# rafayaamirgull/stereo_reconstruction_cv

Hardware: AMD Instinct MI355X
Metric: Mdisparities/s (higher is better)
Workload: dtype int16

## Files before the change

stereo_reconstruction_cv_amd/_lib.py:

```python
from __future__ import annotations

import ctypes as C
import os

_HERE = os.path.dirname(os.path.abspath(__file__))
LIB_PATH = os.environ.get("SGM_HIP_LIB") or os.path.join(_HERE, "csrc", "libsgm_hip.so")

SGM_OK = 0
SGM_TAP_COST, SGM_TAP_AGGR, SGM_TAP_DISP_RAW, SGM_TAP_DISP_MEDIAN = 0, 1, 2, 3
SGM_TAP_CONF_RAW, SGM_TAP_CONF = 4, 5
SGM_TAP_RIGHT_RAW, SGM_TAP_RIGHT = 6, 7
SGM_OPT_KEEP_AGGR, SGM_OPT_PROFILE, SGM_OPT_SCHEDULE, SGM_OPT_SWEEP_ROWS, SGM_OPT_PREPASS_ROWS, SGM_OPT_CHAIN_WGS, SGM_OPT_GROUP_MAX = 0, 1, 2, 3, 5, 6, 7
SGM_OPT_CHANNELS = 8
SGM_OPT_CONFIDENCE = 10
SGM_OPT_RIGHT_VIEW = 11
SGM_OPT_COST = 12
SGM_COST_BT, SGM_COST_CENSUS = 0, 1
SGM_OPT_DEBUG = 4
SGM_OPT_POISON = 9
SGM_DBG_VOXEL_TIGHT_TABLE, SGM_DBG_VOXEL_OTHER_REDUCTION = 1 << 22, 1 << 23
SGM_MAX_STAGES = 32

EXPORTS = (
    "sgm_abi_version", "sgm_device_count", "sgm_last_error", "sgm_create", "sgm_destroy",
    "sgm_set_option", "sgm_geometry", "sgm_compute", "sgm_compute_batch", "sgm_disp_to_float",
    "sgm_reproject", "sgm_valid_mask", "sgm_get_tap", "sgm_get_headroom", "sgm_median3x3", "sgm_filter_speckles", "sgm_compact_points",
    "sgm_compact_points_device", "sgm_compact_points_device_async", "sgm_compute_device", "sgm_check", "sgm_trim",
    "sgm_disp_to_float_device", "sgm_reproject_device", "sgm_valid_mask_device",
    "sgm_pipeline_device", "sgm_pipeline_batch_device", "sgm_synchronize", "sgm_get_stage_times", "sgm_algorithmic_bytes",
    "sgm_init_undistort_rectify_map", "sgm_init_undistort_rectify_map_device",
    "sgm_remap_linear_u8", "sgm_remap_linear_u8_device",
)
CONFIDENCE_EXPORTS = ("sgm_bind_confidence_device",)
RIGHT_EXPORTS = ("sgm_bind_right_device",)
WLS_EXPORTS = ("sgm_wls_weights", "sgm_wls_filter", "sgm_wls_filter_device")
WLS_BATCH_EXPORTS = ("sgm_wls_filter_batch", "sgm_wls_filter_batch_device")
LRC_EXPORTS = ("sgm_lrc_confidence", "sgm_lrc_confidence_device", "sgm_lrc_confidence_batch_device")
VOXEL_EXPORTS = ("sgm_voxel_downsample", "sgm_voxel_downsample_device")
MESH_EXPORTS = ("sgm_mesh_grid", "sgm_mesh_grid_device")


# ... 85 lines not shown
    L.sgm_mesh_grid_device.argtypes = [vp, vp, vp, vp, i32, i32, C.c_float, vp, vp, vp, vp, vp]
    L.sgm_synchronize.argtypes = [vp]
    L.sgm_get_stage_times.argtypes = [vp, C.POINTER(SgmStageTimes)]
    L.sgm_algorithmic_bytes.argtypes = [pp, i32, i32, i32]
    L.sgm_algorithmic_bytes.restype = i64
    L.sgm_init_undistort_rectify_map.argtypes = [vp, vp, vp, i32, vp, vp, i32, i32, i32, vp, vp]
    L.sgm_init_undistort_rectify_map_device.argtypes = [vp, vp, vp, i32, vp, vp, i32, i32, i32, vp, vp]
    L.sgm_remap_linear_u8.argtypes = [vp, vp, i32, i32, i64, i32, vp, vp, i32, i32, vp]
    L.sgm_remap_linear_u8_device.argtypes = [vp, vp, i32, i32, i64, i32, vp, vp, i32, i32, vp, i64]
    L.sgm_debug_plan.argtypes = [pp, i32, i32, i32, i32, i32, i32, i32, i32, C.POINTER(SgmDebugPlan)]
    L.sgm_debug_plan.restype = i32
    L.sgm_debug_plan_opts.argtypes = [pp, i32, i32, i32, i32, i32, i32, i32, i32, i32, i32, C.POINTER(SgmDebugPlan)]
    L.sgm_debug_plan_opts.restype = i32
    L.sgm_debug_plan_cost.argtypes = [pp, i32, i32, i32, i32, i32, i32, i32, i32, i32, i32, i32, C.POINTER(SgmDebugPlan)]
    L.sgm_debug_plan_cost.restype = i32
    L.sgm_debug_uniq_threshold.argtypes = [i32, i32]
    L.sgm_debug_uniq_threshold.restype = i32
    L.sgm_debug_wta_split.argtypes = [pp, i32, i32, i32, i32, i32, i32, i32, i32]
    L.sgm_debug_wta_split.restype = i32
    L.sgm_debug_wta_raw_bytes.argtypes = [vp]
    L.sgm_debug_wta_raw_bytes.restype = C.c_longlong
    L.sgm_debug_wta_select_n.argtypes = [i32, i32, vp, i32, vp]
    L.sgm_debug_wta_select_n.restype = i32
    for name in EXPORTS + CONFIDENCE_EXPORTS + RIGHT_EXPORTS + WLS_EXPORTS + WLS_BATCH_EXPORTS + LRC_EXPORTS + VOXEL_EXPORTS + MESH_EXPORTS:
        fn = getattr(L, name)
        if fn.restype is C.c_int and name not in ("sgm_abi_version", "sgm_device_count"):
            fn.restype = i32
    _lib = L
    return L


def last_error() -> str:
    return (load().sgm_last_error() or b"").decode("utf-8", "replace")


def debug_plan(params: dict, H: int, W: int, channels: int = 1, schedule: int = 1, sweep_rows: int = 0, prepass_rows: int = 0,
               debug: int = 0, frames: int = 1, confidence: int = 0, right_view: int = 0, cost: int = SGM_COST_BT) -> dict:
    out = SgmDebugPlan()
    if cost != SGM_COST_BT:
        rc = load().sgm_debug_plan_cost(C.byref(SgmParams(**params)), H, W, channels, schedule, sweep_rows, prepass_rows, debug,
                                        frames, confidence, right_view, cost, C.byref(out))
    elif confidence or right_view:
        rc = load().sgm_debug_plan_opts(C.byref(SgmParams(**params)), H, W, channels, schedule, sweep_rows, prepass_rows, debug,
                                        frames, confidence, right_view, C.byref(out))
    else:
        rc = load().sgm_debug_plan(C.byref(SgmParams(**params)), H, W, channels, schedule, sweep_rows, prepass_rows, debug, frames,
                                   C.byref(out))
    if rc != SGM_OK:
        raise ValueError(f"sgm_debug_plan failed ({rc}): {last_error()}")
    return {n: getattr(out, n) for n, _ in SgmDebugPlan._fields_}


def debug_wta_split(params: dict, H: int, W: int, schedule: int = 2, sweep_rows: int = 0, debug: int = 0, confidence: int = 0,
                    right_view: int = 0, keep_aggr: int = 0) -> bool:
    rc = load().sgm_debug_wta_split(C.byref(SgmParams(**params)), H, W, schedule, sweep_rows, debug, confidence, right_view, keep_aggr)
    if rc < 0:
        raise ValueError(f"sgm_debug_wta_split failed ({rc}): {last_error()}")
    return bool(rc)
```

stereo_reconstruction_cv_amd/csrc/kernels_sweep.h:

```cpp
#pragma once
#include "kernels_path.h"
#include <type_traits>

namespace sgm {

enum { SWEEP_FIRST = 0, SWEEP_ACCUM = 1, SWEEP_LAST = 2, SWEEP_REDUCE = 3 };

struct SweepArgs {
    int ydir, xdir;
    int R;
    const int16_t *C;
    int16_t *S;
    const int16_t *bndL;
    uint2 *wta;
    int keepS;
    int dbg;
    uint32_t *ctl;
    uint32_t *prog;
    uint32_t *err;
    int nbands;
};

constexpr int CHAIN_MAX_FRAMES = 64;
struct ChainFrames {
    int nf;
    const int16_t *C[CHAIN_MAX_FRAMES];
    int16_t *S[CHAIN_MAX_FRAMES];
    int16_t *bnd[CHAIN_MAX_FRAMES];
    uint32_t *hr[CHAIN_MAX_FRAMES];
    uint4 *raw[CHAIN_MAX_FRAMES];
};
static_assert(sizeof(Geom) + sizeof(SweepArgs) + sizeof(ChainFrames) + 64 <= 4096, "a kernel's arguments must stay within 4 KB");

constexpr int SWEEP_MAX_ROWS = 11;
__host__ __device__ constexpr int sweep_pps(int NP) { return NP == 4 ? 1 : (NP == 1 ? 4 : 2); }
__host__ __device__ constexpr int sweep_ring(int NP) { return 4 * sweep_pps(NP); }

__host__ __device__ constexpr int sweep_slot_dwords(int NP, int NR = 3) { return 64 * NR * NP; }
static inline size_t sweep_lds_bytes(int NP, int R, int NR = 3)
// ... 51 lines not shown
        until(need);
        pending = __hip_atomic_load(word, __ATOMIC_RELAXED, __HIP_MEMORY_SCOPE_AGENT);
    }
    __device__ __forceinline__ void until(uint32_t need)
    {
        if (seen >= need) return;
        uint32_t idle = 0, last = seen;
        for (;;) {
            seen = peek();
            if (seen >= need) break;
            __builtin_amdgcn_s_sleep(8);
            if (seen != last) {
                last = seen;
                idle = 0;
            } else if (++idle > CHAIN_GIVE_UP) {
                if (lane_id() == 0) atomicOr(err, 1u);
                seen = 0x7fffffffu;
                break;
            }
        }
    }
};

#ifndef SGM_CHAIN_HALF_BLOCKS
#define SGM_CHAIN_HALF_BLOCKS 0
#endif
template <int NP, bool PARTIAL, bool CHAIN, int NR = 3>
__device__ __forceinline__ void sweep_loader_wave(const Geom &g, const SweepArgs &a, int band, int lane, uint32_t *lds)
{
    constexpr int LDAUX = CHAIN ? 16 : (SGM_NT_SWEEP_LOADS ? 2 : 0);
    constexpr int PPS = sweep_pps(NP);
    constexpr int RING = sweep_ring(NP);
    constexpr int LB = (CHAIN && SGM_CHAIN_HALF_BLOCKS) ? RING / 2 : RING;
    constexpr int OFF_A = 0, OFF_B = LB % RING;
    static_assert(2 * PPS <= LB && LB % PPS == 0 && RING % LB == 0, "prologue writes 2 * PPS pixels of block 0");
    constexpr int SLOT = sweep_slot_dwords(NP, NR);
    constexpr int ROLE = 64 * NP;
    const int R = a.R;
    int W1 = g.W1;
    const int D = g.D;
    if (CHAIN) asm volatile("" : "+s"(W1));
    const int T = (W1 + PPS - 1) / PPS + 2 * (R - 1);
    const bool active = !PARTIAL || (2 * NP * lane < D);
    const int lane_off = active ? 2 * NP * lane : 0;
    const uint32_t init = active ? (CHAIN ? path_bias(g.P2) : 0u) : SGM_SENT;
    uint32_t *const ring0 = lds + lane * NP;

    const bool has_prev = band > 0 && !(a.dbg & 64);
    Pack<NP> bA[LB][NR], bB[LB][NR];
    const int row_bytes = W1 * NR * D * 2;
    const __amdgpu_buffer_rsrc_t rsrc = __builtin_amdgcn_make_buffer_rsrc(
        (void *)(a.bndL + (int64_t)band * W1 * NR * D), 0, row_bytes, 0x00020000);
    const int voff = lane_off * 2;
    const int px_bytes = NR * D * 2;
    const int pk = a.xdir > 0 ? px_bytes : -px_bytes;
    const int p0 = a.xdir > 0 ? 0 : (W1 - 1) * px_bytes;
    ChainWait cw;
    if (CHAIN && has_prev) {
        cw.word = a.prog + band - 1;
        cw.err = a.err;
    }
    auto lb_t = [&](auto full_c, Pack<NP>(*b)[NR], int k0) {
        constexpr bool FULL = decltype(full_c)::value;
        if (CHAIN) cw.step((uint32_t)min(k0 + LB, W1));
#pragma unroll
        for (int u = 0; u < LB; u++) {
            if (FULL || k0 + u < W1) {
                const int so = p0 + (k0 + u) * pk;
#pragma unroll
                for (int d = 0; d < NR; d++) buf_load<NP, LDAUX>(b[u][d], rsrc, voff, so + d * D * 2);
            }
        }
    };
    auto wb_t = [&](auto full_c, Pack<NP>(*b)[NR], int off, int u, int k) {
        constexpr bool FULL = decltype(full_c)::value;
// ... 363 lines not shown
            load_block_t(part, cB, sB, k0 + PB);
            compute_block_t(part, cA, sA, k0);
            load_block_t(part, cA, sA, k0 + 2 * PB);
            compute_block_t(part, cB, sB, k0 + PB);
        }
    }
    {
        const uint32_t hmax = wave_max_u32(hm) & 0xffffu;
        if (g.hr && lane == 0) headroom_raise(g.hr + 1, hmax);
    }
    if (wave < R - 1) {
        sweep_write_start_state<NP, NR>(mine, W1 % RING, init);
        for (int i = 0; i < 2 * (R - 1 - wave); i++) wg_barrier();
    }
}

template <int NP, bool PARTIAL, int MODE, bool POSW>
__global__ __launch_bounds__(SWEEP_MAX_ROWS * 64 + 64) void k_sweep(Geom g, SweepArgs a)
{
    extern __shared__ __attribute__((aligned(16))) uint32_t lds[];
    const int wave = __builtin_amdgcn_readfirstlane((int)(threadIdx.x >> 6));
    const int lane = threadIdx.x & 63;
    const int band = blockIdx.x;
    if (wave == a.R) sweep_loader_wave<NP, PARTIAL, false>(g, a, band, lane, lds);
    else sweep_compute_wave<NP, PARTIAL, MODE, POSW>(g, a, band, wave, lane, lds);
}

#ifndef SGM_CHAIN_KD
#define SGM_CHAIN_KD 3
#endif
constexpr int CHAIN_KD = SGM_CHAIN_KD;

template <int NP, bool PARTIAL, int NR = 3>
__device__ __forceinline__ void chain_publisher_wave(const Geom &g, const SweepArgs &a, int band, int lane, uint32_t *lds)
{
    constexpr int PPS = sweep_pps(NP);
    constexpr int RING = sweep_ring(NP);
    constexpr int SLOT = sweep_slot_dwords(NP, NR);
    constexpr int ROLE = 64 * NP;
    constexpr int STORES_PER_STEP = NR * PPS * (NP == 4 ? 2 : 1) + 1;
    static_assert(CHAIN_KD * STORES_PER_STEP <= 63, "vmcnt is a 6-bit counter");
    const int R = a.R;
    int W1 = g.W1;
    const int D = g.D;
    asm volatile("" : "+s"(W1));
    const int NS = (W1 + PPS - 1) / PPS;
    const int T = NS + 2 * (R - 1);
    const bool active = !PARTIAL || (2 * NP * lane < D);
    const int lane_off = active ? 2 * NP * lane : 0;
    const bool publishes = band + 1 < a.nbands;
    const uint32_t *const last = lds + lane * NP + R * RING * SLOT;
    const int row_bytes = W1 * NR * D * 2;
    const __amdgpu_buffer_rsrc_t rec = __builtin_amdgcn_make_buffer_rsrc(
        (void *)(a.bndL + (int64_t)(band + 1) * W1 * NR * D), 0, row_bytes, 0x00020000);
    const int voff = lane_off * 2;
    const int px_bytes = NR * D * 2;
    const int pk = a.xdir > 0 ? px_bytes : -px_bytes;
    const int p0 = a.xdir > 0 ? 0 : (W1 - 1) * px_bytes;
    uint32_t *const word = a.prog + band;
    if (!publishes) {
        for (int n = 0; n <= T; n++) wg_barrier();
        return;
    }
    for (int n = 0; n <= T + 1; n++) {
        const int i = n - 2 * (R - 1) - 2;
        if (i >= 0 && i < NS) {
#pragma unroll
            for (int p = 0; p < PPS; p++) {
                const int k = PPS * i + p;
                const uint32_t *s = last + (k % RING) * SLOT;
                Pack<NP> v[NR];
#pragma unroll
                for (int d = 0; d < NR; d++) lds_load<NP>(v[d], s + d * ROLE);
                const int so = k < W1 ? p0 + k * pk : row_bytes;
#pragma unroll
                for (int d = 0; d < NR; d++)
                    if (!PARTIAL || active) buf_store<NP, 16>(v[d], rec, voff, so + d * D * 2);
// ... 2 lines not shown
            Pack<NP> z;
            z.fill(0u);
#pragma unroll
            for (int p = 0; p < NR * PPS; p++)
                if (!PARTIAL || active) buf_store<NP, 16>(z, rec, voff, row_bytes);
        }
        __builtin_amdgcn_s_waitcnt(0x0f70 | ((CHAIN_KD * STORES_PER_STEP) & 15) | (((CHAIN_KD * STORES_PER_STEP) >> 4) << 14));
        const int done = min(max(PPS * (i - CHAIN_KD + 1), 0), W1);
        if (lane == 0) __hip_atomic_store(word, (uint32_t)done, __ATOMIC_RELAXED, __HIP_MEMORY_SCOPE_AGENT);
        if (n <= T) wg_barrier();
    }
    __builtin_amdgcn_s_waitcnt(0x0f70);
    if (lane == 0) __hip_atomic_store(word, (uint32_t)W1, __ATOMIC_RELAXED, __HIP_MEMORY_SCOPE_AGENT);
}

constexpr int CHAIN_MAX_ROWS = 12;
template <int NP, bool PARTIAL, int MODE>
__global__ __launch_bounds__(CHAIN_MAX_ROWS * 64 + 128) void k_sweep_chain(Geom g, SweepArgs a, ChainFrames fr)
{
    extern __shared__ __attribute__((aligned(16))) uint32_t lds[];
    const int wave = __builtin_amdgcn_readfirstlane((int)(threadIdx.x >> 6));
    const int lane = threadIdx.x & 63;
    uint32_t *const ticket = lds + (a.R + 1) * sweep_ring(NP) * sweep_slot_dwords(NP);
    for (;;) {
        if (threadIdx.x == 0) *ticket = atomicAdd(a.ctl, 1u);
        wg_barrier();
        const int tk = __builtin_amdgcn_readfirstlane((int)*ticket);
        if (tk >= a.nbands * fr.nf) break;
        const int f = tk % fr.nf, band = tk / fr.nf;
        a.C = fr.C[f];
        a.S = fr.S[f];
        a.bndL = fr.bnd[f];
        a.prog = a.ctl + 1 + f * a.nbands;
        g.hr = fr.hr[f];
        if constexpr (MODE == SWEEP_REDUCE) a.wta = reinterpret_cast<uint2 *>(fr.raw[f]);
        if (wave == a.R) sweep_loader_wave<NP, PARTIAL, true>(g, a, band, lane, lds);
        else if (wave == a.R + 1) chain_publisher_wave<NP, PARTIAL>(g, a, band, lane, lds);
        else sweep_compute_wave<NP, PARTIAL, MODE, true, 3, true>(g, a, band, wave, lane, lds);
    }
}

template <int NP, bool PARTIAL, int MODE>
__global__ __launch_bounds__(SWEEP_MAX_ROWS * 64 + 64) void k_axis_sweep(Geom g, SweepArgs a)
{
    static_assert(MODE == SWEEP_FIRST || MODE == SWEEP_ACCUM, "the axis-only sweeps have no fused winner-take-all");
    extern __shared__ __attribute__((aligned(16))) uint32_t lds[];
    const int wave = __builtin_amdgcn_readfirstlane((int)(threadIdx.x >> 6));
    const int lane = threadIdx.x & 63;
    const int band = blockIdx.x;
    if (wave == a.R) sweep_loader_wave<NP, PARTIAL, false, 1>(g, a, band, lane, lds);
    else sweep_compute_wave<NP, PARTIAL, MODE, true, 1>(g, a, band, wave, lane, lds);
}

template <int NP, bool PARTIAL, int MODE>
__global__ __launch_bounds__(CHAIN_MAX_ROWS * 64 + 128) void k_axis_chain(Geom g, SweepArgs a, ChainFrames fr)
{
    static_assert(MODE == SWEEP_FIRST || MODE == SWEEP_ACCUM, "the axis-only sweeps have no fused winner-take-all");
    extern __shared__ __attribute__((aligned(16))) uint32_t lds[];
    const int wave = __builtin_amdgcn_readfirstlane((int)(threadIdx.x >> 6));
    const int lane = threadIdx.x & 63;
    uint32_t *const ticket = lds + (a.R + 1) * sweep_ring(NP) * sweep_slot_dwords(NP, 1);
    for (;;) {
        if (threadIdx.x == 0) *ticket = atomicAdd(a.ctl, 1u);
        wg_barrier();
        const int tk = __builtin_amdgcn_readfirstlane((int)*ticket);
        if (tk >= a.nbands * fr.nf) break;
        const int f = tk % fr.nf, band = tk / fr.nf;
        a.C = fr.C[f];
        a.S = fr.S[f];
        a.bndL = fr.bnd[f];
        a.prog = a.ctl + 1 + f * a.nbands;
        g.hr = fr.hr[f];
        if (wave == a.R) sweep_loader_wave<NP, PARTIAL, true, 1>(g, a, band, lane, lds);
        else if (wave == a.R + 1) chain_publisher_wave<NP, PARTIAL, 1>(g, a, band, lane, lds);
        else sweep_compute_wave<NP, PARTIAL, MODE, true, 1, true>(g, a, band, wave, lane, lds);
    }
}

}
```

stereo_reconstruction_cv_amd/csrc/sgm_debug.h:

```cpp
#ifndef SGM_DEBUG_H
#define SGM_DEBUG_H

#define SGM_OPT_DEBUG 4

#define SGM_OPT_POISON 9

enum {
    SGM_DBG_WTA_IN_LAST_PATH = 2,
    SGM_DBG_NO_LANE_GROUPS = 4,
    SGM_DBG_NARROW_VSUM = 8,
    SGM_DBG_PREPASS_3_LAUNCHES = 16,
    SGM_DBG_NO_PREPASS_OVERLAP = 32,
    SGM_DBG_SKIP_BOUNDARY_LOADS = 64,
    SGM_DBG_FORK_PREPASS_EARLY = 128,
    SGM_DBG_INT16_COST = 256,
    SGM_DBG_PREPASS_ONE_CHUNK = 512,
    SGM_DBG_WTA_SEPARATE = 2048,
    SGM_DBG_SMALL_D_RECORD = 8192,
    SGM_DBG_IN_ROW_ON_MAIN_STREAM = 4096,
    SGM_DBG_FIFTH_PATH_AFTER_SWEEP = 65536,
    SGM_DBG_WLS_BATCH_ROWS_SHIFT = 17,
    SGM_DBG_WLS_BATCH_COLS_SHIFT = 20,
    SGM_DBG_VOXEL_TIGHT_TABLE = 1 << 22,
    SGM_DBG_VOXEL_OTHER_REDUCTION = 1 << 23
};

typedef struct {
    int W1, minX1, NP, partial;
    int byte_cost, pix_px, GWc, RBb, vsum_ring;
    int rows4, GWs, chain, R, nbands;
    int fused_prepass, prepass_g, pre_nch, pre_rows, overlap;
    int fused_wta, nvol, path_w_main, speckle;
    int chain_window;
} sgm_debug_plan_t;

#ifdef __cplusplus
extern "C"
#endif
int sgm_debug_plan(const sgm_params *p, int H, int W, int channels, int schedule, int sweep_rows, int prepass_rows,
                   int debug, int frames, sgm_debug_plan_t *out);
#ifdef __cplusplus
extern "C"
#endif
int sgm_debug_plan_opts(const sgm_params *p, int H, int W, int channels, int schedule, int sweep_rows, int prepass_rows,
                        int debug, int frames, int confidence, int right_view, sgm_debug_plan_t *out);
#ifdef __cplusplus
extern "C"
#endif
int sgm_debug_plan_cost(const sgm_params *p, int H, int W, int channels, int schedule, int sweep_rows, int prepass_rows,
                        int debug, int frames, int confidence, int right_view, int cost, sgm_debug_plan_t *out);

#ifdef __cplusplus
extern "C" {
#endif
int sgm_debug_uniq_threshold(int minS, int uniquenessRatio);
int sgm_debug_wta_split(const sgm_params *p, int H, int W, int schedule, int sweep_rows, int debug, int confidence, int right_view,
                        int keep_aggr);
long long sgm_debug_wta_raw_bytes(const sgm_engine *e);
int sgm_debug_wta_select_n(int D, int uniquenessRatio, const uint32_t *raw , int n, uint32_t *wta );
#ifdef __cplusplus
}
#endif

#endif
```

stereo_reconstruction_cv_amd/csrc/sgm_engine.hip:

```cpp
#include "../../include/sgm_hip.h"
#include "sgm_debug.h"

#include <hip/hip_runtime.h>

#include <dlfcn.h>

#include <algorithm>
#include <cmath>
#include <cstdarg>
#include <cstdio>
#include <cstdlib>
#include <cstring>
#include <string>
#include <thread>
#include <vector>

#include "kernels_cost.h"
#include "kernels_census.h"
#include "kernels_path.h"
#include "kernels_post.h"
#include "kernels_rectify.h"
#include "kernels_sweep.h"
#include "kernels_group.h"
#include "kernels_right.h"
// ... 145 lines not shown
        cap = bytes;
        return SGM_OK;
    }
    void release()
    {
        if (p) (void)hipHostFree(p);
        p = nullptr;
        cap = 0;
    }
};

struct Plan {
    bool byte_cost;
    bool pix_px;
    int GWc, RBb;
    bool vsum_ring, vsum_wide;
    int cn;
    bool census;
    bool v1;
    int GWs;
    bool rows4;
    bool chain;
    int npass, R, nbands;
    bool axis;
    int nroles;
    bool prepass_g;
    bool fused_prepass;
    bool pre_plain;
    int pre_nch, pre_rows;
    bool overlap, fork_early;
    bool fused_wta;
    bool wta_split;
    int nvol;
    bool path_w_main, path_w_lines;
    bool speckle;
};

#define SGM_ENGINE_DEVBUFS(BUF, ARR, MAP) \
    BUF(in_left) BUF(in_right)                    \
    BUF(lrec) BUF(rplanes)                        \
    BUF(hsum) BUF(cost) BUF(aggr)                 \
    BUF(aggr2) BUF(aggr3)                         \
    BUF(aggr4) BUF(aggr5)                         \
    BUF(wta)                                      \
    BUF(wta_raw)                                  \
    BUF(bndL) BUF(bndL2)                          \
// ... 349 lines not shown
    hipLaunchKernelGGL((k_sweep_chain<NP, PARTIAL, MODE>), dim3(wgs), dim3((a.R + 2) * 64), lds, st, g, a, fr);
    return SGM_OK;
}
template <int NP, bool PARTIAL>
static int launch_chain_np(const Geom &g, const SweepArgs &a, const ChainFrames &fr, int mode, int wgs, hipStream_t st)
{
    if (mode == SWEEP_FIRST) return launch_chain_one<NP, PARTIAL, SWEEP_FIRST>(g, a, fr, wgs, st);
    if constexpr (!PARTIAL && NP <= 2)
        if (mode == SWEEP_REDUCE) return launch_chain_one<NP, PARTIAL, SWEEP_REDUCE>(g, a, fr, wgs, st);
    if (mode == SWEEP_REDUCE) return set_err(SGM_ERR_INVALID_ARG, "internal: no SWEEP_REDUCE form of this chained sweep");
    return launch_chain_one<NP, PARTIAL, SWEEP_ACCUM>(g, a, fr, wgs, st);
}
static int launch_chain(const Geom &g, const SweepArgs &a, const ChainFrames &fr, int mode, int wgs, hipStream_t st, bool axis = false)
{
    if (int rc = check_sweep_direction(a, mode)) return rc;
    if (axis && mode == SWEEP_REDUCE) return set_err(SGM_ERR_INVALID_ARG, "internal: the axis-only sweeps have no SWEEP_REDUCE form");
    if (axis)
        return with_np(g, [&](auto np, auto part) {
            return mode == SWEEP_FIRST ? launch_axis_chain_one<np, part, SWEEP_FIRST>(g, a, fr, wgs, st)
                                       : launch_axis_chain_one<np, part, SWEEP_ACCUM>(g, a, fr, wgs, st);
        });
    return with_np(g, [&](auto np, auto part) { return launch_chain_np<np, part>(g, a, fr, mode, wgs, st); });
}
static int chain_window(const Geom &g, int R, int nbands, int nf, int override_wgs)
{
    const int pps = sweep_pps(g.NP);
    const int T = (g.W1 + pps - 1) / pps + 2 * (R - 1), lag = 2 * (R - 1) + 17;
    const int per_frame = override_wgs > 0 ? override_wgs : std::max(4, (T + lag - 1) / lag);
    return (int)std::min<int64_t>({(int64_t)per_frame * nf, (int64_t)nbands * nf, 256});
}

static int sweep_rows_for(const Geom &g, int override_rows, int npass, bool chained = false)
{
    int maxR = chained ? CHAIN_MAX_ROWS : SWEEP_MAX_ROWS;
    while (maxR > 1 && sweep_lds_bytes(g.NP, maxR) + 16 > 160 * 1024) maxR--;
    if (chained && override_rows <= 0) return std::max(1, std::min(maxR, g.H));
    const int bands = npass == 2 ? 200 : 240;
    int R = override_rows > 0 ? override_rows : (g.H + bands - 1) / bands;
    if (override_rows <= 0) R = std::max(R, 4);
    return std::max(1, std::min(R, maxR));
}

static int box_columns(int GW) { return 16 * (64 / GW); }

static Plan make_plan(const sgm_engine *e, const Geom &g, int H)
{
// ... 41 lines not shown
    p.wta_split = p.chain && g.mode == 1 && !p.axis && !p.fused_wta && !np_partial(g) && g.NP <= 2 && g.uniq < 100 &&
                  !e->keep_aggr && !e->no_wta_split && !conf && !(dbg & SGM_DBG_WTA_SEPARATE);
    const bool two_vol = g.mode == 0 && !p.fused_wta && !p.v1 && g.D <= 128 && !(dbg & SGM_DBG_NO_LANE_GROUPS) &&
                         !(dbg & SGM_DBG_FIFTH_PATH_AFTER_SWEEP);
    const bool three_vol = two_vol && p.rows4 && !(dbg & SGM_DBG_IN_ROW_ON_MAIN_STREAM);
    const bool five_vol = three_vol && !(dbg & SGM_DBG_SMALL_D_RECORD);
    p.nvol = five_vol ? 5 : three_vol ? 3 : two_vol ? 2 : 1;
    if (p.axis && p.rows4 && !p.v1) {
        p.nvol = 4;
        p.overlap = false;
    }
    p.path_w_main = !p.v1 && g.mode == 0 && p.nvol == 1;
    p.path_w_lines = (dbg & SGM_DBG_NO_LANE_GROUPS) != 0;
    p.speckle = e->params.speckleRange >= 0 && e->params.speckleWindowSize > 0;
    if (g.NP == 8) {
        p.v1 = true;
        p.byte_cost = p.pix_px = p.rows4 = p.chain = p.prepass_g = p.fused_prepass = false;
        p.overlap = p.fork_early = p.path_w_main = false;
        p.GWs = 64;
        p.fused_wta = !conf;
        p.wta_split = false;
        p.nvol = 1;
    }
    return p;
}

static int ensure_speckle_buffers(sgm_engine *e, size_t npx)
{
    int rc;
    if ((rc = e->label.ensure(npx * 4)) || (rc = e->csize.ensure(npx * 4))) return rc;
    return e->rlen.ensure(npx * 4);
}
static size_t chain_ctl_bytes(int nf, int nbands) { return ((size_t)(1 + (size_t)nf * nbands) * 4 + 15) & ~(size_t)15; }

static size_t plan_bytes_held(const sgm_engine *e)
{
    size_t n = 0;
    each_devbuf(e, [&](const DevBuf &b) { n += b.cap; });
    return n;
}
static int ensure_plan_buffers(sgm_engine *e, const Plan &p, int H, int W)
{
    Geom g;
    int rc = normalise(&e->params, H, W, &g);
    if (rc) return rc;
    e->g = g;
    e->H = H;
    e->W = W;
    const size_t npx = (size_t)H * W;
    const size_t vol = (size_t)std::max<int64_t>(g.rowsz, 0) * H * sizeof(int16_t);
    if ((rc = e->lrec.ensure(npx * 8 * p.cn + (debug_alloc_mode() ? 0 : 64)))) return rc;
    if ((rc = e->rplanes.ensure(p.census ? npx * 8 : npx * 6 * p.cn))) return rc;
    if (vol) {
        if (!p.byte_cost && (rc = e->hsum.ensure(vol))) return rc;
        if ((rc = e->cost.ensure(vol))) return rc;
        if ((rc = e->aggr.ensure(vol))) return rc;
        DevBuf *more[] = {&e->aggr2, &e->aggr3, &e->aggr4, &e->aggr5};
        for (int k = 1; k < p.nvol; k++)
            if ((rc = more[k - 1]->ensure(vol))) return rc;
    }
    if ((rc = e->wta.ensure(npx * 8))) return rc;
    if (p.wta_split && (rc = e->wta_raw.ensure(npx * 16))) return rc;
    if ((rc = e->disp_raw.ensure(npx * 2))) return rc;
    if ((rc = e->disp_med.ensure(npx * 2))) return rc;
    for (SideMap *m : {&e->conf, &e->right})
        if (m->on && ((rc = m->raw.ensure(npx * m->bpp)) || (rc = m->fin.ensure(npx * m->bpp)))) return rc;
    if (e->right.on && g.W1 > 0 && (rc = e->rrec.ensure((size_t)H * g.W1 * 8))) return rc;
    if ((rc = e->headroom.ensure(8))) return rc;
    e->g.hr = (uint32_t *)e->headroom.p;
    if (g.W1 > 0 && !p.v1 && p.nbands > 1 && p.nvol < 4) {
        const size_t bnd_bytes = (size_t)p.nbands * g.W1 * p.nroles * g.D * 2;
        if ((rc = e->bndL.ensure(bnd_bytes))) return rc;
        if (!p.chain) {
            if (p.npass == 2 && (rc = e->bndL2.ensure(bnd_bytes))) return rc;
            if (!p.axis) {
                const size_t st_bytes = (size_t)2 * 3 * g.W1 * g.D * 2;
                if ((rc = e->pstate.ensure(st_bytes))) return rc;
                if (p.npass == 2 && (rc = e->pstate2.ensure(st_bytes))) return rc;
            }
        }
    }
    if (p.speckle && (rc = ensure_speckle_buffers(e, npx))) return rc;
    if (p.chain) {
        if ((rc = e->chain_ctl.ensure(chain_ctl_bytes(1, p.nbands)))) return rc;
        if (!e->chain_err.p) {
            if ((rc = e->chain_err.ensure(16))) return rc;
            HIP_TRY(hipMemsetAsync(e->chain_err.p, 0, 16, e->stream));
        }
    }
    return SGM_OK;
}

static int run_speckles(sgm_engine *e, int16_t *d_img, int H, int W, int newVal, int maxSpeckleSize, int maxDiff)
{
    const size_t npx = (size_t)H * W;
    int rc;
    if ((rc = ensure_speckle_buffers(e, npx))) return rc;
    int *label = (int *)e->label.p, *csz = (int *)e->csize.p, *rlen = (int *)e->rlen.p;
    hipStream_t st = e->stream;
    dim3 g2((W + 255) / 256, H);
    hipLaunchKernelGGL(k_ccl_rows, dim3(H), dim3(64), 0, st, (const int16_t *)d_img, label, rlen, csz, W, newVal, maxDiff);
    hipLaunchKernelGGL(k_ccl_merge, g2, dim3(256), 0, st, (const int16_t *)d_img, label, H, W, newVal, maxDiff);
    hipLaunchKernelGGL(k_ccl_count, g2, dim3(256), 0, st, (const int16_t *)d_img, label, (const int *)rlen, csz, H, W, newVal, maxDiff);
    hipLaunchKernelGGL(k_ccl_apply, g2, dim3(256), 0, st, d_img, label, (const int *)csz, H, W, newVal, maxDiff, maxSpeckleSize);
    KCHECK();
    return SGM_OK;
}

__global__ void k_fill_i16(int16_t *p, int64_t n, int16_t v)
{
// ... 368 lines not shown
    int16_t *S = (int16_t *)e->aggr.p;
    uint2 *wta = (uint2 *)e->wta.p;
    int rc;
    if (p.nvol == 4)
        return run_stage(e, "paths4", st, [&] {
            int16_t *const Sv[5] = {S, (int16_t *)e->aggr2.p, (int16_t *)e->aggr3.p, (int16_t *)e->aggr4.p, nullptr};
            launch_axis_paths4(g, p.GWs, C, Sv, st);
            return 1;
        });
    if (p.overlap && p.fork_early && (rc = fork_prepass_up(e, p))) return rc;
    for (int pass = 0; pass < p.npass; pass++) {
        const int ydir = pass == 0 ? 1 : -1, xdir = ydir;
        int16_t *bl = (int16_t *)(pass == 0 ? e->bndL.p : e->bndL2.p);
        if (p.nbands > 1 && !(p.overlap && pass == 1) && !p.chain && p.nvol != 5) {
            rc = run_stage(e, pass == 0 ? "prepass_dn" : "prepass_up", st, [&] { return launch_prepass(e, p, xdir, ydir, bl, st); });
            if (rc) return rc;
        }
        if (p.overlap && pass == 0 && !p.fork_early && (rc = fork_prepass_up(e, p))) return rc;
        if (p.overlap && pass == 1) {
            HIP_TRY(hipStreamWaitEvent(st, e->ev_join, 0));
            stage_break(e);
        }
        const bool last = pass == p.npass - 1 && g.mode == 1 && p.fused_wta && !p.rows4;
        SweepArgs a{ydir, xdir, p.R, C, S, (const int16_t *)bl, wta, e->keep_aggr, e->debug, nullptr, nullptr, nullptr, p.nbands};
        ChainFrames fr;
        if (p.chain) {
            fr.nf = 1;
            fr.C[0] = C;
            fr.S[0] = S;
            fr.bnd[0] = (int16_t *)e->bndL.p;
            fr.hr[0] = g.hr;
            fr.raw[0] = (uint4 *)e->wta_raw.p;
            a.ctl = (uint32_t *)e->chain_ctl.p;
            a.err = (uint32_t *)e->chain_err.p;
            HIP_TRY(hipMemsetAsync(e->chain_ctl.p, 0, chain_ctl_bytes(1, p.nbands), st));
            stage_break(e);
        }
        const char *name = p.nvol == 5 ? "paths5" : p.chain ? (pass == 0 ? "chain_dn" : "chain_up")
                                                             : (pass == 0 ? "sweep_dn" : (p.fused_wta ? "sweep_up_wta" : "sweep_up"));
        rc = run_stage(e, name, st, [&]() -> int {
            if (p.nvol == 5) {
                int16_t *const Sv[5] = {S, (int16_t *)e->aggr2.p, (int16_t *)e->aggr3.p, (int16_t *)e->aggr4.p, (int16_t *)e->aggr5.p};
                launch_paths5(g, p.GWs, C, Sv, st);
            } else if (p.rows4) {
                launch_vert3(g, p.GWs, pass == 0, xdir, C, S, bl, p.prepass_g ? 1 : 0, st);
                if (p.nvol < 3) launch_rows_grouped(g, g.H, p.GWs, xdir, PATH_ACCUM, C, S, 1, wta, st);
            } else if (p.chain) {
// ... 323 lines not shown
    out->nvol = p.nvol;
    out->path_w_main = p.path_w_main;
    out->speckle = p.speckle;
    out->chain_window = p.chain && g.W1 > 0 ? chain_window(g, p.R, p.nbands, std::max(frames, 1), 0) : 0;
    return SGM_OK;
}

int sgm_debug_plan(const sgm_params *params, int H, int W, int channels, int schedule, int sweep_rows, int prepass_rows,
                   int debug, int frames, sgm_debug_plan_t *out)
{
    return debug_plan_on(params, H, W, channels, schedule, sweep_rows, prepass_rows, debug, frames, 0, 0, SGM_COST_BT, out);
}

int sgm_debug_plan_opts(const sgm_params *params, int H, int W, int channels, int schedule, int sweep_rows, int prepass_rows,
                        int debug, int frames, int confidence, int right_view, sgm_debug_plan_t *out)
{
    return debug_plan_on(params, H, W, channels, schedule, sweep_rows, prepass_rows, debug, frames, confidence, right_view, SGM_COST_BT, out);
}

int sgm_debug_plan_cost(const sgm_params *params, int H, int W, int channels, int schedule, int sweep_rows, int prepass_rows,
                        int debug, int frames, int confidence, int right_view, int cost, sgm_debug_plan_t *out)
{
    return debug_plan_on(params, H, W, channels, schedule, sweep_rows, prepass_rows, debug, frames, confidence, right_view, cost, out);
}

int sgm_debug_uniq_threshold(int minS, int uniquenessRatio)
{
    if (minS < 0 || minS > SGM_MAX_COST || uniquenessRatio < 0 || uniquenessRatio > 99) return -1;
    return (int)uniq_t1((uint32_t)minS, uniq_recip(uniquenessRatio));
}
int sgm_debug_wta_split(const sgm_params *params, int H, int W, int schedule, int sweep_rows, int debug, int confidence, int right_view,
                        int keep_aggr)
{
    if (!params) return set_err(SGM_ERR_INVALID_ARG, "params is null");
    if (H <= 0 || W < 2 || W > 32767 || H > 32767) return set_err(SGM_ERR_INVALID_ARG, "bad shape H=%d W=%d", H, W);
    sgm_engine e;
    e.params = *params;
    int rc;
    if ((rc = sgm_set_option(&e, SGM_OPT_SCHEDULE, schedule)) || (rc = sgm_set_option(&e, SGM_OPT_SWEEP_ROWS, sweep_rows)) ||
        (rc = sgm_set_option(&e, SGM_OPT_DEBUG, debug)) || (rc = sgm_set_option(&e, SGM_OPT_CONFIDENCE, confidence)) ||
        (rc = sgm_set_option(&e, SGM_OPT_RIGHT_VIEW, right_view)) || (rc = sgm_set_option(&e, SGM_OPT_KEEP_AGGR, keep_aggr)))
        return rc;
    Geom g;
    if ((rc = normalise(&e.params, H, W, &g))) return rc;
    return make_plan(&e, g, H).wta_split ? 1 : 0;
}
// ... 482 lines not shown
    ~BatchGuard()
    {
        e->hr_accumulate = false;
        e->in_batch = false;
        for (sgm_engine *q : e->group) q->hr_accumulate = false;
        if (ok) return;
        (void)hipStreamSynchronize(e->stream);
        for (sgm_engine *q : e->group) (void)hipStreamSynchronize(q->stream);
        if (e->copy_in) (void)hipStreamSynchronize(e->copy_in);
        if (e->copy_out) (void)hipStreamSynchronize(e->copy_out);
    }
};

static int run_group(sgm_engine *e, sgm_engine *const *eng, int n, const Plan &pl, const PairIO *io, int H, int W, int64_t stride_bytes,
                     const double Q[16], const hipEvent_t *in_ready, const hipEvent_t *in_used, const hipEvent_t *out_done)
{
    int rc;
    HIP_TRY(hipEventRecord(e->ev_group, e->stream));
    for (int k = 1; k < n; k++) HIP_TRY(hipStreamWaitEvent(eng[k]->stream, e->ev_group, 0));
    for (int k = 0; k < n; k++) {
        if (in_ready && in_ready[k]) HIP_TRY(hipStreamWaitEvent(eng[k]->stream, in_ready[k], 0));
        if ((rc = run_compute(eng[k], io[k], H, W, stride_bytes, PH_PRE))) return rc;
        const Plan &q = eng[k]->plan;
        if (!q.chain || q.R != pl.R || q.nbands != pl.nbands || q.axis != pl.axis || q.wta_split != pl.wta_split)
            return set_err(SGM_ERR_HIP, "internal: a pair of a chained group did not plan the group's chained sweep");
        if (in_used && in_used[k]) HIP_TRY(hipEventRecord(in_used[k], eng[k]->stream));
    }
    const Geom &g = e->g;
    const int R = pl.R, nbands = pl.nbands, npass = pl.npass;
    const size_t ctl_bytes = chain_ctl_bytes(n, nbands);
    if ((rc = e->chain_ctl.ensure(ctl_bytes))) return rc;
    for (int k = 1; k < n; k++) {
        HIP_TRY(hipEventRecord(eng[k]->ev_done, eng[k]->stream));
        HIP_TRY(hipStreamWaitEvent(e->stream, eng[k]->ev_done, 0));
    }
    stage_break(e);
    ChainFrames fr;
    fr.nf = n;
    for (int k = 0; k < n; k++) {
        fr.C[k] = (const int16_t *)eng[k]->cost.p;
        fr.S[k] = (int16_t *)eng[k]->aggr.p;
        fr.bnd[k] = (int16_t *)eng[k]->bndL.p;
        fr.hr[k] = eng[k]->g.hr;
        fr.raw[k] = (uint4 *)eng[k]->wta_raw.p;
    }
    for (int pass = 0; pass < npass; pass++) {
        const int ydir = pass == 0 ? 1 : -1;
        SweepArgs a{ydir, ydir, R, nullptr, nullptr, nullptr, nullptr, 0, e->debug, (uint32_t *)e->chain_ctl.p, nullptr,
                    (uint32_t *)e->chain_err.p, nbands};
        HIP_TRY(hipMemsetAsync(e->chain_ctl.p, 0, ctl_bytes, e->stream));
        stage_break(e);
        if ((rc = stage_begin(e, pass == 0 ? "chain_dn" : "chain_up"))) return rc;
        const int cm = pass == 0 ? SWEEP_FIRST : (pl.wta_split ? SWEEP_REDUCE : SWEEP_ACCUM);
        if ((rc = launch_chain(g, a, fr, cm, chain_window(g, R, nbands, n, e->chain_wgs), e->stream, pl.axis))) return rc;
        KCHECK();
        if ((rc = stage_end(e, 1))) return rc;
    }
    HIP_TRY(hipEventRecord(e->ev_group, e->stream));
    for (int k = 0; k < n; k++) {
        if (k > 0) HIP_TRY(hipStreamWaitEvent(eng[k]->stream, e->ev_group, 0));
        if (out_done && k >= 3 && out_done[k - 3]) HIP_TRY(hipStreamWaitEvent(eng[k]->stream, out_done[k - 3], 0));
        if ((rc = run_compute(eng[k], io[k], H, W, stride_bytes, PH_POST))) return rc;
        if ((rc = run_float_xyz(eng[k], (const int16_t *)io[k].disp_i16, H, W, Q, io[k].disp_f32, io[k].xyz_f32))) return rc;
        if (out_done && out_done[k]) HIP_TRY(hipEventRecord(out_done[k], eng[k]->stream));
    }
    for (int k = 1; k < n; k++) {
        HIP_TRY(hipEventRecord(eng[k]->ev_done, eng[k]->stream));
        HIP_TRY(hipStreamWaitEvent(e->stream, eng[k]->ev_done, 0));
    }
    stage_break(e);
    return SGM_OK;
}
// ... 1076 lines not shown
```

Measured before the change: 347,300.

## Use a small ring of boundary handoff records in chained sweep

In the chained sweep, the per-band boundary handoff records are now stored in a ring of a few rows (default 2) indexed by band modulo ring, instead of one row per band. This shrinks the bndL buffer and keeps the handoff working set small enough that it may stay resident in cache. Because the record row is reused, correctness depends on the chain's progress synchronisation keeping a consumer from reading a row after it has been overwritten. The change also adds a debug query for the planned byte sizes and narrows the dbg field to 16 bits.

```diff
diff --git a/stereo_reconstruction_cv_amd/_lib.py b/stereo_reconstruction_cv_amd/_lib.py
--- a/stereo_reconstruction_cv_amd/_lib.py
+++ b/stereo_reconstruction_cv_amd/_lib.py
@@ -17,6 +17,7 @@
 SGM_OPT_COST = 12
 SGM_COST_BT, SGM_COST_CENSUS = 0, 1
 SGM_OPT_DEBUG = 4
+SGM_DBG_HANDOFF_RING_SHIFT = 24
 SGM_OPT_POISON = 9
 SGM_DBG_VOXEL_TIGHT_TABLE, SGM_DBG_VOXEL_OTHER_REDUCTION = 1 << 22, 1 << 23
 SGM_MAX_STAGES = 32
@@ -148,6 +149,9 @@
     L.sgm_debug_wta_raw_bytes.restype = C.c_longlong
     L.sgm_debug_wta_select_n.argtypes = [i32, i32, vp, i32, vp]
     L.sgm_debug_wta_select_n.restype = i32
+    if hasattr(L, "sgm_debug_handoff_ring"):
+        L.sgm_debug_handoff_ring.argtypes = [pp, i32, i32, i32, i32, i32, C.POINTER(C.c_longlong), C.POINTER(C.c_longlong)]
+        L.sgm_debug_handoff_ring.restype = i32
     for name in EXPORTS + CONFIDENCE_EXPORTS + RIGHT_EXPORTS + WLS_EXPORTS + WLS_BATCH_EXPORTS + LRC_EXPORTS + VOXEL_EXPORTS + MESH_EXPORTS:
         fn = getattr(L, name)
         if fn.restype is C.c_int and name not in ("sgm_abi_version", "sgm_device_count"):
@@ -183,3 +187,11 @@
     if rc < 0:
         raise ValueError(f"sgm_debug_wta_split failed ({rc}): {last_error()}")
     return bool(rc)
+
+
+def debug_handoff_ring(params: dict, H: int, W: int, schedule: int = 2, sweep_rows: int = 0, debug: int = 0) -> dict:
+    rec, tot = C.c_longlong(0), C.c_longlong(0)
+    rc = load().sgm_debug_handoff_ring(C.byref(SgmParams(**params)), H, W, schedule, sweep_rows, debug, C.byref(rec), C.byref(tot))
+    if rc < 0:
+        raise ValueError(f"sgm_debug_handoff_ring failed ({rc}): {last_error()}")
+    return dict(ring=rc, record_bytes=rec.value, engine_bytes=tot.value)
diff --git a/stereo_reconstruction_cv_amd/csrc/kernels_sweep.h b/stereo_reconstruction_cv_amd/csrc/kernels_sweep.h
--- a/stereo_reconstruction_cv_amd/csrc/kernels_sweep.h
+++ b/stereo_reconstruction_cv_amd/csrc/kernels_sweep.h
@@ -14,7 +14,8 @@
     const int16_t *bndL;
     uint2 *wta;
     int keepS;
-    int dbg;
+    uint16_t dbg;
+    uint16_t ring;
     uint32_t *ctl;
     uint32_t *prog;
     uint32_t *err;
@@ -112,11 +113,23 @@
     }
 };
 
+__device__ __forceinline__ int chain_row(int band, int ring)
+{
+uint32_t b = (uint32_t)band; asm volatile("" : "+v"(b)); return (int)(b % (uint32_t)ring);
+}
+template <typename T>
+__device__ __forceinline__ T *uniform_ptr(T *p)
+{
+    const uint64_t v = (uint64_t)p;
+    return (T *)(((uint64_t)(uint32_t)__builtin_amdgcn_readfirstlane((int)(v >> 32)) << 32) |
+                 (uint32_t)__builtin_amdgcn_readfirstlane((int)(uint32_t)v));
+}
+
 #ifndef SGM_CHAIN_HALF_BLOCKS
 #define SGM_CHAIN_HALF_BLOCKS 0
 #endif
 template <int NP, bool PARTIAL, bool CHAIN, int NR = 3>
-__device__ __forceinline__ void sweep_loader_wave(const Geom &g, const SweepArgs &a, int band, int lane, uint32_t *lds)
+__device__ __forceinline__ void sweep_loader_wave(const Geom &g, const SweepArgs &a, int band, int rec_row, int lane, uint32_t *lds)
 {
     constexpr int LDAUX = CHAIN ? 16 : (SGM_NT_SWEEP_LOADS ? 2 : 0);
     constexpr int PPS = sweep_pps(NP);
@@ -139,8 +152,9 @@
     const bool has_prev = band > 0 && !(a.dbg & 64);
     Pack<NP> bA[LB][NR], bB[LB][NR];
     const int row_bytes = W1 * NR * D * 2;
-    const __amdgpu_buffer_rsrc_t rsrc = __builtin_amdgcn_make_buffer_rsrc(
-        (void *)(a.bndL + (int64_t)band * W1 * NR * D), 0, row_bytes, 0x00020000);
+    const int16_t *rec_base = a.bndL + (int64_t)rec_row * W1 * NR * D;
+    if constexpr (CHAIN) rec_base = uniform_ptr(rec_base);
+    const __amdgpu_buffer_rsrc_t rsrc = __builtin_amdgcn_make_buffer_rsrc((void *)rec_base, 0, row_bytes, 0x00020000);
     const int voff = lane_off * 2;
     const int px_bytes = NR * D * 2;
     const int pk = a.xdir > 0 ? px_bytes : -px_bytes;
@@ -550,7 +564,7 @@
     const int wave = __builtin_amdgcn_readfirstlane((int)(threadIdx.x >> 6));
     const int lane = threadIdx.x & 63;
     const int band = blockIdx.x;
-    if (wave == a.R) sweep_loader_wave<NP, PARTIAL, false>(g, a, band, lane, lds);
+    if (wave == a.R) sweep_loader_wave<NP, PARTIAL, false>(g, a, band, band, lane, lds);
     else sweep_compute_wave<NP, PARTIAL, MODE, POSW>(g, a, band, wave, lane, lds);
 }
 
@@ -560,7 +574,7 @@
 constexpr int CHAIN_KD = SGM_CHAIN_KD;
 
 template <int NP, bool PARTIAL, int NR = 3>
-__device__ __forceinline__ void chain_publisher_wave(const Geom &g, const SweepArgs &a, int band, int lane, uint32_t *lds)
+__device__ __forceinline__ void chain_publisher_wave(const Geom &g, const SweepArgs &a, int band, int rec_row, int lane, uint32_t *lds)
 {
     constexpr int PPS = sweep_pps(NP);
     constexpr int RING = sweep_ring(NP);
@@ -580,7 +594,7 @@
     const uint32_t *const last = lds + lane * NP + R * RING * SLOT;
     const int row_bytes = W1 * NR * D * 2;
     const __amdgpu_buffer_rsrc_t rec = __builtin_amdgcn_make_buffer_rsrc(
-        (void *)(a.bndL + (int64_t)(band + 1) * W1 * NR * D), 0, row_bytes, 0x00020000);
+        (void *)uniform_ptr(a.bndL + (int64_t)rec_row * W1 * NR * D), 0, row_bytes, 0x00020000);
     const int voff = lane_off * 2;
     const int px_bytes = NR * D * 2;
     const int pk = a.xdir > 0 ? px_bytes : -px_bytes;
@@ -629,20 +643,27 @@
     const int wave = __builtin_amdgcn_readfirstlane((int)(threadIdx.x >> 6));
     const int lane = threadIdx.x & 63;
     uint32_t *const ticket = lds + (a.R + 1) * sweep_ring(NP) * sweep_slot_dwords(NP);
+    const uint32_t dbg_ring = (uint32_t)a.dbg | ((uint32_t)a.ring << 16);
     for (;;) {
         if (threadIdx.x == 0) *ticket = atomicAdd(a.ctl, 1u);
         wg_barrier();
         const int tk = __builtin_amdgcn_readfirstlane((int)*ticket);
         if (tk >= a.nbands * fr.nf) break;
         const int f = tk % fr.nf, band = tk / fr.nf;
+        {
+            uint32_t w = dbg_ring;
+            asm volatile("" : "+s"(w));
+            a.dbg = (uint16_t)w;
+            a.ring = (uint16_t)(w >> 16);
+        }
         a.C = fr.C[f];
         a.S = fr.S[f];
         a.bndL = fr.bnd[f];
         a.prog = a.ctl + 1 + f * a.nbands;
         g.hr = fr.hr[f];
         if constexpr (MODE == SWEEP_REDUCE) a.wta = reinterpret_cast<uint2 *>(fr.raw[f]);
-        if (wave == a.R) sweep_loader_wave<NP, PARTIAL, true>(g, a, band, lane, lds);
-        else if (wave == a.R + 1) chain_publisher_wave<NP, PARTIAL>(g, a, band, lane, lds);
+        if (wave == a.R) sweep_loader_wave<NP, PARTIAL, true>(g, a, band, chain_row(band, a.ring), lane, lds);
+        else if (wave == a.R + 1) chain_publisher_wave<NP, PARTIAL>(g, a, band, chain_row(band + 1, a.ring), lane, lds);
         else sweep_compute_wave<NP, PARTIAL, MODE, true, 3, true>(g, a, band, wave, lane, lds);
     }
 }
@@ -655,7 +676,7 @@
     const int wave = __builtin_amdgcn_readfirstlane((int)(threadIdx.x >> 6));
     const int lane = threadIdx.x & 63;
     const int band = blockIdx.x;
-    if (wave == a.R) sweep_loader_wave<NP, PARTIAL, false, 1>(g, a, band, lane, lds);
+    if (wave == a.R) sweep_loader_wave<NP, PARTIAL, false, 1>(g, a, band, band, lane, lds);
     else sweep_compute_wave<NP, PARTIAL, MODE, true, 1>(g, a, band, wave, lane, lds);
 }
 
@@ -667,19 +688,26 @@
     const int wave = __builtin_amdgcn_readfirstlane((int)(threadIdx.x >> 6));
     const int lane = threadIdx.x & 63;
     uint32_t *const ticket = lds + (a.R + 1) * sweep_ring(NP) * sweep_slot_dwords(NP, 1);
+    const uint32_t dbg_ring = (uint32_t)a.dbg | ((uint32_t)a.ring << 16);
     for (;;) {
         if (threadIdx.x == 0) *ticket = atomicAdd(a.ctl, 1u);
         wg_barrier();
         const int tk = __builtin_amdgcn_readfirstlane((int)*ticket);
         if (tk >= a.nbands * fr.nf) break;
         const int f = tk % fr.nf, band = tk / fr.nf;
+        {
+            uint32_t w = dbg_ring;
+            asm volatile("" : "+s"(w));
+            a.dbg = (uint16_t)w;
+            a.ring = (uint16_t)(w >> 16);
+        }
         a.C = fr.C[f];
         a.S = fr.S[f];
         a.bndL = fr.bnd[f];
         a.prog = a.ctl + 1 + f * a.nbands;
         g.hr = fr.hr[f];
-        if (wave == a.R) sweep_loader_wave<NP, PARTIAL, true, 1>(g, a, band, lane, lds);
-        else if (wave == a.R + 1) chain_publisher_wave<NP, PARTIAL, 1>(g, a, band, lane, lds);
+        if (wave == a.R) sweep_loader_wave<NP, PARTIAL, true, 1>(g, a, band, chain_row(band, a.ring), lane, lds);
+        else if (wave == a.R + 1) chain_publisher_wave<NP, PARTIAL, 1>(g, a, band, chain_row(band + 1, a.ring), lane, lds);
         else sweep_compute_wave<NP, PARTIAL, MODE, true, 1, true>(g, a, band, wave, lane, lds);
     }
 }
diff --git a/stereo_reconstruction_cv_amd/csrc/sgm_debug.h b/stereo_reconstruction_cv_amd/csrc/sgm_debug.h
--- a/stereo_reconstruction_cv_amd/csrc/sgm_debug.h
+++ b/stereo_reconstruction_cv_amd/csrc/sgm_debug.h
@@ -22,7 +22,8 @@
     SGM_DBG_WLS_BATCH_ROWS_SHIFT = 17,
     SGM_DBG_WLS_BATCH_COLS_SHIFT = 20,
     SGM_DBG_VOXEL_TIGHT_TABLE = 1 << 22,
-    SGM_DBG_VOXEL_OTHER_REDUCTION = 1 << 23
+    SGM_DBG_VOXEL_OTHER_REDUCTION = 1 << 23,
+    SGM_DBG_HANDOFF_RING_SHIFT = 24
 };
 
 typedef struct {
@@ -51,6 +52,12 @@
                         int debug, int frames, int confidence, int right_view, int cost, sgm_debug_plan_t *out);
 
 #ifdef __cplusplus
+extern "C"
+#endif
+int sgm_debug_handoff_ring(const sgm_params *p, int H, int W, int schedule, int sweep_rows, int debug, long long *record_bytes,
+                           long long *engine_bytes);
+
+#ifdef __cplusplus
 extern "C" {
 #endif
 int sgm_debug_uniq_threshold(int minS, int uniquenessRatio);
diff --git a/stereo_reconstruction_cv_amd/csrc/sgm_engine.hip b/stereo_reconstruction_cv_amd/csrc/sgm_engine.hip
--- a/stereo_reconstruction_cv_amd/csrc/sgm_engine.hip
+++ b/stereo_reconstruction_cv_amd/csrc/sgm_engine.hip
@@ -191,6 +191,7 @@
     bool rows4;
     bool chain;
     int npass, R, nbands;
+    int ring;
     bool axis;
     int nroles;
     bool prepass_g;
@@ -586,6 +587,7 @@
         });
     return with_np(g, [&](auto np, auto part) { return launch_chain_np<np, part>(g, a, fr, mode, wgs, st); });
 }
+constexpr int CHAIN_RING_DEFAULT = 2;
 static int chain_window(const Geom &g, int R, int nbands, int nf, int override_wgs)
 {
     const int pps = sweep_pps(g.NP);
@@ -673,6 +675,8 @@
         p.wta_split = false;
         p.nvol = 1;
     }
+    const int ring_field = (dbg >> SGM_DBG_HANDOFF_RING_SHIFT) & 7;
+    p.ring = !p.chain ? 0 : ring_field == 7 ? p.nbands : std::min(ring_field ? ring_field : CHAIN_RING_DEFAULT, p.nbands);
     return p;
 }
 
@@ -690,8 +694,18 @@
     each_devbuf(e, [&](const DevBuf &b) { n += b.cap; });
     return n;
 }
-static int ensure_plan_buffers(sgm_engine *e, const Plan &p, int H, int W)
-{
+static size_t handoff_record_bytes(const Plan &p, const Geom &g)
+{
+    return (size_t)(p.chain ? p.ring : p.nbands) * g.W1 * p.nroles * g.D * 2;
+}
+static int ensure_plan_buffers(sgm_engine *e, const Plan &p, int H, int W, size_t *planned = nullptr)
+{
+    if (planned) *planned = 0;
+    auto need = [&](DevBuf &b, size_t bytes) -> int {
+        if (!planned) return b.ensure(bytes);
+        *planned += bytes;
+        return SGM_OK;
+    };
     Geom g;
     int rc = normalise(&e->params, H, W, &g);
     if (rc) return rc;
@@ -700,43 +714,46 @@
     e->W = W;
     const size_t npx = (size_t)H * W;
     const size_t vol = (size_t)std::max<int64_t>(g.rowsz, 0) * H * sizeof(int16_t);
-    if ((rc = e->lrec.ensure(npx * 8 * p.cn + (debug_alloc_mode() ? 0 : 64)))) return rc;
-    if ((rc = e->rplanes.ensure(p.census ? npx * 8 : npx * 6 * p.cn))) return rc;
+    if ((rc = need(e->lrec, npx * 8 * p.cn + (debug_alloc_mode() ? 0 : 64)))) return rc;
+    if ((rc = need(e->rplanes, p.census ? npx * 8 : npx * 6 * p.cn))) return rc;
     if (vol) {
-        if (!p.byte_cost && (rc = e->hsum.ensure(vol))) return rc;
-        if ((rc = e->cost.ensure(vol))) return rc;
-        if ((rc = e->aggr.ensure(vol))) return rc;
+        if (!p.byte_cost && (rc = need(e->hsum, vol))) return rc;
+        if ((rc = need(e->cost, vol))) return rc;
+        if ((rc = need(e->aggr, vol))) return rc;
         DevBuf *more[] = {&e->aggr2, &e->aggr3, &e->aggr4, &e->aggr5};
         for (int k = 1; k < p.nvol; k++)
-            if ((rc = more[k - 1]->ensure(vol))) return rc;
-    }
-    if ((rc = e->wta.ensure(npx * 8))) return rc;
-    if (p.wta_split && (rc = e->wta_raw.ensure(npx * 16))) return rc;
-    if ((rc = e->disp_raw.ensure(npx * 2))) return rc;
-    if ((rc = e->disp_med.ensure(npx * 2))) return rc;
+            if ((rc = need(*more[k - 1], vol))) return rc;
+    }
+    if ((rc = need(e->wta, npx * 8))) return rc;
+    if (p.wta_split && (rc = need(e->wta_raw, npx * 16))) return rc;
+    if ((rc = need(e->disp_raw, npx * 2))) return rc;
+    if ((rc = need(e->disp_med, npx * 2))) return rc;
     for (SideMap *m : {&e->conf, &e->right})
-        if (m->on && ((rc = m->raw.ensure(npx * m->bpp)) || (rc = m->fin.ensure(npx * m->bpp)))) return rc;
-    if (e->right.on && g.W1 > 0 && (rc = e->rrec.ensure((size_t)H * g.W1 * 8))) return rc;
-    if ((rc = e->headroom.ensure(8))) return rc;
+        if (m->on && ((rc = need(m->raw, npx * m->bpp)) || (rc = need(m->fin, npx * m->bpp)))) return rc;
+    if (e->right.on && g.W1 > 0 && (rc = need(e->rrec, (size_t)H * g.W1 * 8))) return rc;
+    if ((rc = need(e->headroom, 8))) return rc;
     e->g.hr = (uint32_t *)e->headroom.p;
     if (g.W1 > 0 && !p.v1 && p.nbands > 1 && p.nvol < 4) {
-        const size_t bnd_bytes = (size_t)p.nbands * g.W1 * p.nroles * g.D * 2;
-        if ((rc = e->bndL.ensure(bnd_bytes))) return rc;
+        const size_t bnd_bytes = handoff_record_bytes(p, g);
+        if ((rc = need(e->bndL, bnd_bytes))) return rc;
         if (!p.chain) {
-            if (p.npass == 2 && (rc = e->bndL2.ensure(bnd_bytes))) return rc;
+            if (p.npass == 2 && (rc = need(e->bndL2, bnd_bytes))) return rc;
             if (!p.axis) {
                 const size_t st_bytes = (size_t)2 * 3 * g.W1 * g.D * 2;
-                if ((rc = e->pstate.ensure(st_bytes))) return rc;
-                if (p.npass == 2 && (rc = e->pstate2.ensure(st_bytes))) return rc;
+                if ((rc = need(e->pstate, st_bytes))) return rc;
+                if (p.npass == 2 && (rc = need(e->pstate2, st_bytes))) return rc;
             }
         }
     }
-    if (p.speckle && (rc = ensure_speckle_buffers(e, npx))) return rc;
+    if (p.speckle) {
+        if (planned) *planned += 3 * npx * 4;
+        else if ((rc = ensure_speckle_buffers(e, npx))) return rc;
+    }
     if (p.chain) {
-        if ((rc = e->chain_ctl.ensure(chain_ctl_bytes(1, p.nbands)))) return rc;
+        if ((rc = need(e->chain_ctl, chain_ctl_bytes(1, p.nbands)))) return rc;
         if (!e->chain_err.p) {
-            if ((rc = e->chain_err.ensure(16))) return rc;
-            HIP_TRY(hipMemsetAsync(e->chain_err.p, 0, 16, e->stream));
+            if ((rc = need(e->chain_err, 16))) return rc;
+            if (!planned) HIP_TRY(hipMemsetAsync(e->chain_err.p, 0, 16, e->stream));
         }
     }
     return SGM_OK;
@@ -1151,7 +1168,7 @@
             stage_break(e);
         }
         const bool last = pass == p.npass - 1 && g.mode == 1 && p.fused_wta && !p.rows4;
-        SweepArgs a{ydir, xdir, p.R, C, S, (const int16_t *)bl, wta, e->keep_aggr, e->debug, nullptr, nullptr, nullptr, p.nbands};
+        SweepArgs a{ydir, xdir, p.R, C, S, (const int16_t *)bl, wta, e->keep_aggr, (uint16_t)(e->debug & 0xffff), (uint16_t)p.ring, nullptr, nullptr, nullptr, p.nbands};
         ChainFrames fr;
         if (p.chain) {
             fr.nf = 1;
@@ -1521,6 +1538,28 @@
                         int debug, int frames, int confidence, int right_view, int cost, sgm_debug_plan_t *out)
 {
     return debug_plan_on(params, H, W, channels, schedule, sweep_rows, prepass_rows, debug, frames, confidence, right_view, cost, out);
+}
+
+int sgm_debug_handoff_ring(const sgm_params *params, int H, int W, int schedule, int sweep_rows, int debug, long long *record_bytes,
+                           long long *engine_bytes)
+{
+    if (!params) return set_err(SGM_ERR_INVALID_ARG, "params is null");
+    if (H <= 0 || W < 2 || W > 32767 || H > 32767) return set_err(SGM_ERR_INVALID_ARG, "bad shape H=%d W=%d", H, W);
+    sgm_engine e;
+    e.params = *params;
+    int rc;
+    if ((rc = sgm_set_option(&e, SGM_OPT_SCHEDULE, schedule)) || (rc = sgm_set_option(&e, SGM_OPT_SWEEP_ROWS, sweep_rows)) ||
+        (rc = sgm_set_option(&e, SGM_OPT_DEBUG, debug)))
+        return rc;
+    Geom g;
+    if ((rc = normalise(&e.params, H, W, &g))) return rc;
+    const Plan p = make_plan(&e, g, H);
+    size_t planned = 0;
+    if ((rc = ensure_plan_buffers(&e, p, H, W, &planned))) return rc;
+    const bool has_record = g.W1 > 0 && !p.v1 && p.nbands > 1 && p.nvol < 4;
+    if (record_bytes) *record_bytes = has_record ? (long long)handoff_record_bytes(p, g) : 0;
+    if (engine_bytes) *engine_bytes = (long long)planned;
+    return p.chain ? p.ring : 0;
 }
 
 int sgm_debug_uniq_threshold(int minS, int uniquenessRatio)
@@ -2049,7 +2088,7 @@
         if (in_ready && in_ready[k]) HIP_TRY(hipStreamWaitEvent(eng[k]->stream, in_ready[k], 0));
         if ((rc = run_compute(eng[k], io[k], H, W, stride_bytes, PH_PRE))) return rc;
         const Plan &q = eng[k]->plan;
-        if (!q.chain || q.R != pl.R || q.nbands != pl.nbands || q.axis != pl.axis || q.wta_split != pl.wta_split)
+        if (!q.chain || q.R != pl.R || q.nbands != pl.nbands || q.ring != pl.ring || q.axis != pl.axis || q.wta_split != pl.wta_split)
             return set_err(SGM_ERR_HIP, "internal: a pair of a chained group did not plan the group's chained sweep");
         if (in_used && in_used[k]) HIP_TRY(hipEventRecord(in_used[k], eng[k]->stream));
     }
@@ -2073,8 +2112,8 @@
     }
     for (int pass = 0; pass < npass; pass++) {
         const int ydir = pass == 0 ? 1 : -1;
-        SweepArgs a{ydir, ydir, R, nullptr, nullptr, nullptr, nullptr, 0, e->debug, (uint32_t *)e->chain_ctl.p, nullptr,
-                    (uint32_t *)e->chain_err.p, nbands};
+        SweepArgs a{ydir, ydir, R, nullptr, nullptr, nullptr, nullptr, 0, (uint16_t)(e->debug & 0xffff), (uint16_t)pl.ring,
+                    (uint32_t *)e->chain_ctl.p, nullptr, (uint32_t *)e->chain_err.p, nbands};
         HIP_TRY(hipMemsetAsync(e->chain_ctl.p, 0, ctl_bytes, e->stream));
         stage_break(e);
         if ((rc = stage_begin(e, pass == 0 ? "chain_dn" : "chain_up"))) return rc;
```

Result: slower. 343,800 (-1.0%).
